# bdaiinstitute/vlfm

Hardware: AMD Instinct MI355X
Metric: env-steps/s (VLM+value-map update), 640x480 RGB-D (higher is better)
Workload: dtype f16 ViT-g (f32 accumulate) + f32 Q-Former (split-f16, 22-bit); f32 confidence + f64 value maps; 1 GPU; configs[1] step x resident envs: BLIP-2 ITC + ValueMap+ObstacleMap+sort_waypoints; envs_per_gpu=256, global_envs=256, map=1000x1000 @ 20 px/m, parallelism=env-sharded x1, tuned_gemms=True, vit_gemm=hip:fc1, attention=hip

## Files before the change

### include/vlfm_amd.h

```cpp
#ifndef VLFM_AMD_H
#define VLFM_AMD_H

#include <stddef.h>
#include <stdint.h>

#ifdef __cplusplus
extern "C" {
#endif

typedef enum {
    VLFM_OK = 0,
    VLFM_ERR_INVALID = -1,
    VLFM_ERR_OUTSIDE_MAP = -2,
    VLFM_ERR_INDEX = -3,
    VLFM_ERR_HIP = -4,
    VLFM_ERR_CAPACITY = -5
} vlfm_status;

enum { VLFM_FUSE_DEFAULT = 0, VLFM_FUSE_REPLACE = 1, VLFM_FUSE_EQUAL_WEIGHTING = 2 };

const char* vlfm_last_error(void);
int vlfm_abi_version(void);

int vlfm_profile_enable(int on);
// ... 127 lines not shown
                                int out_dtype, int patch_size, void* stream);

int vlfm_itc_head_batched(const float* d_proj, int batch, int n_query, int proj_dim,
                          const float* d_text, float* d_out, void* stream);

#define VLFM_ITC_MAX_PROMPTS 8
int vlfm_itc_head_multi(const float* d_proj, int batch, int n_query, int proj_dim, const float* d_text_table, int n_text,
                        const int32_t* d_text_index, int n_prompts, float* d_out, void* stream);

int vlfm_layernorm_bias_f16(const void* d_x, const float* d_channel_bias, const void* d_gamma, const void* d_beta,
                            void* d_y, int rows, int dim, float eps, void* stream);

int vlfm_vit_attention_f16(const void* d_qkv, void* d_out, int batch, int tokens, int heads, int head_dim, float scale,
                           void* stream);

int vlfm_gemm_f16_nt(const void* d_x, const void* d_w, const void* d_bias, void* d_c, int m, int n, int k, int epilogue,
                     void* stream);

int vlfm_gemm_f16_pair_f32_nt(const void* d_x, const void* d_w_pair, const void* d_bias_f32, void* d_out, int m, int n_out, int k,
                              void* stream);

int vlfm_qformer_cross_attention_f32(const void* d_q, const void* d_kv_blocks, void* d_out, int batch, int tokens, int queries,
                                     int heads, int k_block0, int v_block0, int m_total, float scale, void* stream);

int vlfm_gemm_f16_tile_order(int m, int n, int group_m, int* out, int capacity_pairs);
int vlfm_gemm_f16_work_items(int m, int n, int grid, int* out, int capacity_pairs);

int vlfm_split_f32_to_f16_pair(const float* d_src, void* d_hi, void* d_lo, long long count, int* d_overflow, void* stream);
int vlfm_gemm_f32_nt(const float* d_x, const float* d_w, const float* d_bias, const float* d_residual, float* d_c, int m, int n,
                     int k, int activation, int precision, const void* d_w_hi, const void* d_w_lo, int* d_overflow, void* stream);


int vlfm_layernorm_rows_f32(const float* d_x, const float* d_gamma, const float* d_beta, float* d_out, int batch, int height,
                            int width, int channels, int window, float eps, void* stream);
int vlfm_window_reverse_add_f32(float* d_x, const float* d_windows, int batch, int height, int width, int channels, int window,
                                void* stream);
int vlfm_dwconv3x3_nhwc_f32(const float* d_x, const float* d_w9c, const float* d_bias, float* d_out, int batch, int height, int width,
                            int channels, void* stream);
int vlfm_window_attention_f32(const float* d_qkv, const float* d_bias_t, float* d_out, long long windows, int tokens, int heads,
                              float scale, void* stream);
int vlfm_layernorm_rows_shifted_f32(const float* d_x, const float* d_gamma, const float* d_beta, float* d_out, int batch, int height,
                                    int width, int channels, int window, float eps, int shift, int pad_zero, void* stream);
int vlfm_window_reverse_add_shifted_f32(float* d_x, const float* d_windows, int batch, int height, int width, int channels, int window,
                                        int shift, void* stream);
int vlfm_window_attention_masked_f32(const float* d_qkv, const float* d_bias_t, const float* d_mask_t, int windows_per_image, float* d_out,
                                     long long windows, int tokens, int heads, float scale, void* stream);
// ... 254 lines not shown
```

### vlfm_amd/_lib.py

```python
from __future__ import annotations

import ctypes
import os
import subprocess
from typing import Optional

_HERE = os.path.dirname(os.path.abspath(__file__))
LIB_PATH = os.path.join(_HERE, "libvlfm_amd.so")
SOURCES = ["value_map.hip", "depth_ingest.hip", "depth_holes.hip", "obstacle_map.hip", "vlm_ops.hip", "vit_attention.hip", "qformer_attention.hip", "detect_ops.hip", "object_cloud.hip", "cloud_query.hip", "gemm_f16.hip", "gemm_f32.hip", "conv_nhwc.hip", "sam_ops.hip", "map_render.hip", "jpeg_codec.hip", "jpeg_entropy.hip", "jpeg_decode.hip", "world_render.hip", "depth_sensor.hip", "depth_filter.hip", "geodesic.hip", "map_planner.hip", "lattice_geodesic.hip", "host.cpp"]

VLFM_OK = 0
VLFM_ERR_INVALID = -1
VLFM_ERR_OUTSIDE_MAP = -2
VLFM_ERR_INDEX = -3
VLFM_ERR_HIP = -4
VLFM_ERR_CAPACITY = -5

FUSION_TYPES = {"default": 0, "replace": 1, "equal_weighting": 2}


class VmPose(ctypes.Structure):
    _fields_ = [("inv_affine", ctypes.c_double * 6), ("row0", ctypes.c_int32), ("col0", ctypes.c_int32),
                ("env", ctypes.c_int32), ("reserved", ctypes.c_int32)]


class IngestParams(ctypes.Structure):
    _fields_ = [("tf", ctypes.c_double * 12), ("depth_scale", ctypes.c_float), ("depth_offset", ctypes.c_float),
                ("depth_max", ctypes.c_float), ("reserved0", ctypes.c_float), ("fx", ctypes.c_double),
                ("fy", ctypes.c_double), ("min_height", ctypes.c_double), ("max_height", ctypes.c_double),
                ("env", ctypes.c_int32), ("scatter", ctypes.c_int32)]


# ... 70 lines not shown
    if os.path.exists(LIB_PATH) and all(os.path.getmtime(LIB_PATH) >= os.path.getmtime(o) for o in objs):
        return LIB_PATH
    cmd = ["hipcc", "--offload-arch=gfx950", "-shared", "-fPIC", "-o", LIB_PATH] + objs
    if verbose:
        print(" ".join(cmd), flush=True)
    subprocess.check_call(cmd)
    return LIB_PATH


_lib: Optional[ctypes.CDLL] = None


def lib() -> ctypes.CDLL:
    global _lib
    if _lib is None:
        if not os.path.exists(LIB_PATH):
            raise ImportError(
                f"{LIB_PATH} is missing: build it with `python -c 'import __graft_entry__ as g; g.build()'` "
                "(hipcc --offload-arch=gfx950).  vlfm_amd has no CPU fallback.")
        L = ctypes.CDLL(LIB_PATH)
        vp, ci, cd = ctypes.c_void_p, ctypes.c_int, ctypes.c_double
        L.vlfm_last_error.restype = ctypes.c_char_p
        L.vlfm_abi_version.restype = ci
        L.vlfm_profile_enable.argtypes = [ci]
        L.vlfm_host_wait_mode.argtypes = [ci]
        L.vlfm_profile_read.argtypes = [ctypes.c_char_p, ctypes.POINTER(cd), ctypes.POINTER(ci)]
        L.vlfm_value_map_pose_params.argtypes = [vp, vp, vp, ci, ci, ci, ci, vp, ctypes.POINTER(ci)]
        L.vlfm_cone_template_host.argtypes = [cd, cd, ci, cd, vp, ci, vp, ci, ctypes.POINTER(ci)]
        L.vlfm_tan_table_host.argtypes = [cd, ci, vp]
        L.vlfm_disc_rows_host.argtypes = [ci, vp]
        L.vlfm_cone_template_build.argtypes = [vp, vp, ci, ci, vp, vp, vp]
        L.vlfm_depth_ingest_batched.argtypes = [vp, ci, ci, ci, vp, vp, vp, ci, ci, vp, vp, vp, vp, vp]
        L.vlfm_selftest_div_exact.argtypes = [vp, ci, cd, vp, vp]
        L.vlfm_hole_scratch_bytes.argtypes = [ci, ci, ci, ci, ci]
        L.vlfm_hole_scratch_bytes.restype = ctypes.c_size_t
        L.vlfm_fill_small_holes_batched.argtypes = [vp, vp, ci, ci, ci, cd, vp, ctypes.c_size_t, ci, ci, vp, vp, vp, vp,
                                                    ci, vp, vp]
        L.vlfm_depth_scatter_holes_batched.argtypes = [vp, ci, ci, ci, vp, vp, vp, vp, ci, ci, vp, vp, vp]
        L.vlfm_fill_small_holes_rig_batched.argtypes = [vp, vp, ci, ci, ci, cd, vp, ctypes.c_size_t, ci, ci, vp, vp, vp, vp,
                                                        ci, vp, vp, ci, vp]
        L.vlfm_depth_scatter_holes_rig_batched.argtypes = [vp, ci, ci, ci, vp, vp, vp, vp, ci, ci, vp, vp, vp, vp]
        L.vlfm_layernorm_bias_f16.argtypes = [vp, vp, vp, vp, vp, ci, ci, ctypes.c_float, vp]
        L.vlfm_vit_attention_f16.argtypes = [vp, vp, ci, ci, ci, ci, ctypes.c_float, vp]
        L.vlfm_gemm_f16_nt.argtypes = [vp, vp, vp, vp, ci, ci, ci, ci, vp]
        L.vlfm_gemm_f16_pair_f32_nt.argtypes = [vp, vp, vp, vp, ci, ci, ci, vp]
        L.vlfm_qformer_cross_attention_f32.argtypes = [vp, vp, vp, ci, ci, ci, ci, ci, ci, ci, ctypes.c_float, vp]
        L.vlfm_gemm_f32_nt.argtypes = [vp, vp, vp, vp, vp, ci, ci, ci, ci, ci, vp, vp, vp, vp]
        L.vlfm_split_f32_to_f16_pair.argtypes = [vp, vp, vp, ctypes.c_longlong, vp, vp]
        L.vlfm_layernorm_rows_f32.argtypes = [vp, vp, vp, vp, ci, ci, ci, ci, ci, ctypes.c_float, vp]
        L.vlfm_window_reverse_add_f32.argtypes = [vp, vp, ci, ci, ci, ci, ci, vp]
        L.vlfm_dwconv3x3_nhwc_f32.argtypes = [vp, vp, vp, vp, ci, ci, ci, ci, vp]
        L.vlfm_window_attention_f32.argtypes = [vp, vp, vp, ctypes.c_longlong, ci, ci, ctypes.c_float, vp]
        L.vlfm_layernorm_rows_shifted_f32.argtypes = [vp, vp, vp, vp, ci, ci, ci, ci, ci, ctypes.c_float, ci, ci, vp]
        L.vlfm_window_reverse_add_shifted_f32.argtypes = [vp, vp, ci, ci, ci, ci, ci, ci, vp]
        L.vlfm_window_attention_masked_f32.argtypes = [vp, vp, vp, ci, vp, ctypes.c_longlong, ci, ci, ctypes.c_float, vp]
        L.vlfm_maxpool2x2_nhwc_f16.argtypes = [vp, vp, ci, ci, ci, ci, vp]
        L.vlfm_conv_nhwc_tile.argtypes = [ci, ci, ci, ci, ctypes.POINTER(ci), ctypes.POINTER(ci)]
        L.vlfm_conv_nhwc_f16.argtypes = [vp, vp, vp, vp, vp, ci, ci, ci, ci, ci, ci, ci, ci, ci, ci, vp]
        L.vlfm_value_map_update_fused_batched.argtypes = [vp, ci, vp, vp, vp, ci, vp, vp, ci, vp, vp, ci, ci, ci, cd, cd,
                                                          ci, ci, vp, vp, vp, vp, vp]
        L.vlfm_value_map_update_rig_batched.argtypes = [vp, ci, vp, vp, vp, ci, ci, ci, vp, vp, vp, ci, ci, ci, ci, ci, vp, vp,
                                                        vp, vp]
        L.vlfm_value_map_sort_waypoints_batched.argtypes = [vp, ci, ci, vp, ci, ci, vp, ci, vp, vp]
        L.vlfm_resample_coeffs_host.argtypes = [ci, ci, vp, vp, ci, ctypes.POINTER(ci)]
        L.vlfm_resample_coeffs_filter_host.argtypes = [ci, ci, ci, vp, vp, ci, ctypes.POINTER(ci)]
        L.vlfm_preprocess_sam_batched.argtypes = [vp, ci, ci, ci, ci, ci, vp, vp, ci, vp, vp, ci, vp, vp, ci, vp, vp, vp]
        L.vlfm_preprocess_rgb_batched.argtypes = [vp, ci, ci, ci, ci, vp, vp, ci, vp, vp, ci, vp, vp, vp, vp, ci, ci, vp]
        L.vlfm_itc_head_batched.argtypes = [vp, ci, ci, ci, vp, vp, vp]
        L.vlfm_itc_head_multi.argtypes = [vp, ci, ci, ci, vp, ci, vp, ci, vp, vp]
# ... 127 lines not shown
```

### vlfm_amd/csrc/host.cpp

```cpp
#include <cmath>
#include <cstdint>
#include <cstring>
#include <mutex>
#include <string>

#include "../../include/vlfm_amd.h"
#include "status.h"

namespace vlfm {
static thread_local std::string g_last_error;
void set_last_error(const char* msg) { g_last_error = msg ? msg : ""; }
}

extern "C" const char* vlfm_last_error(void) { return vlfm::g_last_error.c_str(); }
extern "C" int vlfm_abi_version(void) { return 28; }

namespace {

const double kPi = 3.141592653589793238462643383279502884;

inline long round_half_even(double v) { return std::lrint(v); }

float sin_deg_table(int deg) {
    static float tab[451];
    static std::once_flag once;
    std::call_once(once, [] {
        for (int i = 0; i <= 450; i++) tab[i] = (float)(std::round(std::sin(i * kPi / 180.0) * 1e7) / 1e7);
    });
    return tab[deg];
}

}

extern "C" int vlfm_value_map_pose_params(const double* h_tf, const double* h_yaw, const int32_t* h_env, int n,
                                          int map_size, int pixels_per_meter, int template_size,
                                          vlfm_vm_pose* h_out, int* bad_index) {
    if (!h_tf || !h_out || n < 0 || map_size <= 0 || template_size <= 0)
        return vlfm::fail(VLFM_ERR_INVALID, "value_map_pose_params: bad argument");
// ... 255 lines not shown
```

### vlfm_amd/csrc/qformer_attention.hip

```cpp
#include <hip/hip_runtime.h>
#include <stdint.h>

#include "../../include/vlfm_amd.h"
#include "mfma.h"
#include "profile.h"
#include "status.h"

namespace vlfm {

constexpr int QA_ROWB = 256;
constexpr int QA_MERGE_REGS = 34;
constexpr int QA_MERGE = 3 * QA_MERGE_REGS * 64 * 4;
constexpr int QA_MAX_T = 257, QA_MAX_Q = 32;

struct QaArgs {
    const float* q;
    const float* kv;
    float* out;
    int B, T, Q, heads, k_block0, v_block0, M_total;
    int rows_pad;
    float scale_log2e;
};

struct QaKernel {
    const QaArgs& a;
    unsigned char* smem;
    lds_ptr lds;
    int lane, wave, col, g, voff;

    __device__ QaKernel(const QaArgs& a_, unsigned char* smem_) : a(a_), smem(smem_), lds((lds_ptr)smem_) {
        lane = threadIdx.x & 63;
        wave = __builtin_amdgcn_readfirstlane(threadIdx.x >> 6);
        col = lane & 31;
        g = lane >> 5;
        voff = a.rows_pad * QA_ROWB;
    }
    __device__ inline const unsigned char* block(int block0, int b, int h) const {
        return reinterpret_cast<const unsigned char*>(a.kv + ((size_t)(block0 + h) * (size_t)a.M_total + (size_t)b * (size_t)a.T) * 64);
    }
    __device__ inline void issue_k(const unsigned char* kg, int row0, int n_ins) const {
        const int r4 = lane >> 4, p = lane & 15;
        for (int ins = 0; ins < n_ins; ins++) {
            const int row = row0 + 4 * ins + r4, src_row = min(row, a.T - 1);
            const int dst = __builtin_amdgcn_readfirstlane((row0 + 4 * ins) * QA_ROWB);
            __builtin_amdgcn_global_load_lds((gbl_ptr)(kg + (size_t)src_row * QA_ROWB + ((p ^ (row & 15)) << 4)), lds + dst, 16, 0, 0);
        }
    }
    __device__ inline void issue_v(const unsigned char* vg, int row0, int n_ins) const {
        const int r4 = lane >> 4, p = lane & 15;
        for (int ins = 0; ins < n_ins; ins++) {
            const int row = row0 + 4 * ins + r4, src_row = min(row, a.T - 1);
            const int dst = __builtin_amdgcn_readfirstlane(voff + (row0 + 4 * ins) * QA_ROWB);
            __builtin_amdgcn_global_load_lds((gbl_ptr)(vg + (size_t)src_row * QA_ROWB + ((p ^ (((row >> 2) & 1) << 3)) << 4)),
                                             lds + dst, 16, 0, 0);
        }
    }
    __device__ inline void issue_rows(const unsigned char* kg, const unsigned char* vg, int row0, int n_ins) const {
        issue_k(kg, row0, n_ins);
        issue_v(vg, row0, n_ins);
    }
    __device__ inline void load_q(int b, int h, float (&qn)[32]) const {
        const float* src = a.q + ((size_t)b * a.Q + min(col, a.Q - 1)) * ((size_t)a.heads * 64) + (size_t)h * 64 + 32 * g;
#pragma unroll
        for (int c = 0; c < 8; c++) {
            const floatx4 v = *reinterpret_cast<const floatx4*>(src + 4 * c);
            qn[4 * c] = v[0]; qn[4 * c + 1] = v[1]; qn[4 * c + 2] = v[2]; qn[4 * c + 3] = v[3];
        }
    }
};

__device__ __forceinline__ void qa_item(int w, int heads, int& b, int& h) {
    const int xcd = w & 7, idx = w >> 3;
    b = (idx / heads) * 8 + xcd;
    h = idx % heads;
}

__global__ __launch_bounds__(256) void qformer_cross_attention_kernel(QaArgs a) {
    extern __shared__ __attribute__((aligned(16))) unsigned char smem[];
    QaKernel k(a, smem);
    const int lane = k.lane, wave = k.wave, col = k.col, g = k.g;
    const int n_full = a.T >> 5, n_left = a.T & 31, left_wave = n_full & 3, left_ins = (n_left + 3) >> 2;
    const int stride = gridDim.x;
    const int moff = 2 * k.voff;
    int w = blockIdx.x, b, h;
    qa_item(w, a.heads, b, h);
// ... 132 lines not shown
                }
            }
            if (col < a.Q) {
                const float inv = 1.0f / l;
                float* orow = a.out + ((size_t)b * a.Q + col) * ((size_t)a.heads * 64) + (size_t)h * 64 + 4 * g;
#pragma unroll
                for (int q4 = 0; q4 < 4; q4++) {
                    const floatx4 s0 = {o0[4 * q4] * inv, o0[4 * q4 + 1] * inv, o0[4 * q4 + 2] * inv, o0[4 * q4 + 3] * inv};
                    const floatx4 s1 = {o1[4 * q4] * inv, o1[4 * q4 + 1] * inv, o1[4 * q4 + 2] * inv, o1[4 * q4 + 3] * inv};
                    *reinterpret_cast<floatx4*>(orow + 8 * q4) = s0;
                    *reinterpret_cast<floatx4*>(orow + 32 + 8 * q4) = s1;
                }
            }
            wait_lgkmcnt0();
        }
        asm volatile("" ::: "memory");
        __builtin_amdgcn_s_barrier();
        asm volatile("" ::: "memory");
        if (!more) break;
        w = nw; b = nb; h = nh;
    }
}

}

using namespace vlfm;

extern "C" int vlfm_qformer_cross_attention_f32(const void* d_q, const void* d_kv_blocks, void* d_out, int batch, int tokens,
                                                int queries, int heads, int k_block0, int v_block0, int m_total, float scale,
                                                void* stream) {
    if (batch == 0) return VLFM_OK;
    if (!d_q || !d_kv_blocks || !d_out || batch < 0 || tokens < 1 || tokens > QA_MAX_T || queries < 1 || queries > QA_MAX_Q || heads < 1 ||
        k_block0 < 0 || v_block0 < 0 || (long long)batch * tokens > (long long)m_total)
        return fail(VLFM_ERR_INVALID, "qformer_cross_attention_f32: head width 64, 1-32 queries, 1-257 tokens, batch * tokens <= m_total");
    if ((((uintptr_t)d_q | (uintptr_t)d_kv_blocks | (uintptr_t)d_out) & 15) != 0)
        return fail(VLFM_ERR_INVALID, "qformer_cross_attention_f32: pointers must be 16-byte aligned");
    QaArgs a;
    a.q = (const float*)d_q; a.kv = (const float*)d_kv_blocks; a.out = (float*)d_out;
    a.B = batch; a.T = tokens; a.Q = queries; a.heads = heads; a.k_block0 = k_block0; a.v_block0 = v_block0; a.M_total = m_total;
    a.rows_pad = (tokens + 3) & ~3;
    a.scale_log2e = scale * 1.4426950408889634f;
    const size_t lds = 2 * (size_t)a.rows_pad * QA_ROWB + QA_MERGE;
    const void* fn = reinterpret_cast<const void*>(qformer_cross_attention_kernel);
    static LdsOptIn opt;
    if (!opt.ensure(fn, lds)) return fail(VLFM_ERR_HIP, "qformer_cross_attention_f32: cannot opt in to the LDS size");
    const long long items = (long long)((batch + 7) / 8) * 8 * heads;
    const int n_cu = device_cu_count() & ~7;
    const dim3 grid((unsigned)(items < n_cu ? items : n_cu)), block(256);
    VLFM_TIMED("qformer_cross_attention_kernel", stream);
    VLFM_KLAUNCH(qformer_cross_attention_kernel, grid, block, lds, stream, a);
    return check_launch("qformer_cross_attention_kernel");
}
```

### vlfm_amd/vlm/blip2itm.py

```python
from __future__ import annotations

import hashlib
import math
import os
import re
from dataclasses import dataclass
from typing import Dict, List, Optional, Sequence, Tuple

import numpy as np
import torch
import torch.nn as nn
import torch.nn.functional as F


@dataclass
class Blip2ITCConfig:
    image_size: int = 224
    patch_size: int = 14
    v_hidden: int = 1408
    v_layers: int = 39
    v_heads: int = 16
    v_mlp: int = 6144
    v_ln_eps: float = 1e-6
    q_hidden: int = 768
# ... 162 lines not shown
def _qlinear(x: torch.Tensor, lin_w: torch.Tensor, lin_b, act=None, residual=None) -> torch.Tensor:
    from . import ops

    if (x.is_cuda and x.dtype == torch.float32 and lin_w.dtype == torch.float32 and not torch.is_grad_enabled()
            and x.numel() // x.shape[-1] >= QFORMER_SPLIT_MIN_ROWS and ops.linear_f32_supported(x, lin_w)):
        return ops.linear_f32(x, lin_w, lin_b, act=act, residual=residual, precision="split", owner="blip2")
    y = F.linear(x, lin_w, lin_b)
    if act == "gelu":
        y = F.gelu(y)
    return y if residual is None else y + residual


class _BertAttention(nn.Module):
    def __init__(self, hidden: int, kv_hidden: int, heads: int, eps: float):
        super().__init__()
        self.heads = heads
        self.query = nn.Linear(hidden, hidden)
        self.key = nn.Linear(kv_hidden, hidden)
        self.value = nn.Linear(kv_hidden, hidden)
        self.dense = nn.Linear(hidden, hidden)
        self.LayerNorm = nn.LayerNorm(hidden, eps=eps)
        self._kv_split = None
        self._qkv_fused = None

    def _project_kv_f16(self, kv16: torch.Tensor) -> Tuple[torch.Tensor, torch.Tensor]:
        if self._kv_split is None or self._kv_split[0].device != kv16.device:
            w1, w2, w3 = _exact_split3(torch.cat([self.key.weight, self.value.weight]))
            bias = torch.cat([self.key.bias, self.value.bias]).detach().float()
            self._kv_split = (w1.t(), w2.t(), w3.t(), bias)
        o = _split_gemm(kv16.reshape(-1, kv16.shape[-1]), self._kv_split[:3], self._kv_split[3])
        o = o.view(*kv16.shape[:-1], -1)
        hid = self.key.out_features
        return o[..., :hid], o[..., hid:]

    def forward(self, x: torch.Tensor, kv: Optional[torch.Tensor] = None, mask: Optional[torch.Tensor] = None,
                kv_proj: Optional[Tuple[torch.Tensor, torch.Tensor]] = None, kv_blocks=None) -> torch.Tensor:
        b, n, d = x.shape
        h = self.heads
        if kv_blocks is not None:
            from . import ops

            blocks, tokens, k_block0, v_block0 = kv_blocks
            q = _qlinear(x, self.query.weight, self.query.bias).contiguous()
            a = ops.qformer_cross_attention(q, blocks, tokens, h, k_block0, v_block0, (d // h) ** -0.5)
            return self.LayerNorm(_qlinear(a, self.dense.weight, self.dense.bias, residual=x))
        if kv_proj is not None:
            q = _qlinear(x, self.query.weight, self.query.bias).view(b, n, h, d // h).transpose(1, 2)
            k = kv_proj[0].reshape(b, -1, h, d // h).transpose(1, 2)
            v = kv_proj[1].reshape(b, -1, h, d // h).transpose(1, 2)
        elif kv is None and x.is_cuda and not self.training:
            if self._qkv_fused is None or self._qkv_fused[0].device != x.device or self._qkv_fused[0].dtype != x.dtype:
                self._qkv_fused = (torch.cat([self.query.weight, self.key.weight, self.value.weight]).detach(),
                                   torch.cat([self.query.bias, self.key.bias, self.value.bias]).detach())
            qkv = _qlinear(x, *self._qkv_fused).view(b, n, 3, h, d // h).permute(2, 0, 3, 1, 4)
            q, k, v = qkv[0], qkv[1], qkv[2]
        else:
            q = self.query(x).view(b, n, h, d // h).transpose(1, 2)
            if kv is not None and kv.dtype == torch.float16 and kv.is_cuda and self.key.weight.dtype == torch.float32:
                k, v = self._project_kv_f16(kv)
                src_len = kv.shape[1]
            else:
                src = x if kv is None else kv.to(x.dtype)
                k, v, src_len = self.key(src), self.value(src), src.shape[1]
            k = k.reshape(b, src_len, h, d // h).transpose(1, 2)
            v = v.reshape(b, src_len, h, d // h).transpose(1, 2)
        a = F.scaled_dot_product_attention(q, k, v, attn_mask=mask)
        return self.LayerNorm(_qlinear(a.transpose(1, 2).reshape(b, n, d), self.dense.weight, self.dense.bias,
                                       residual=x))


class _BertFFN(nn.Module):
    def __init__(self, hidden: int, inter: int, eps: float):
        super().__init__()
        self.up = nn.Linear(hidden, inter)
        self.down = nn.Linear(inter, hidden)
        self.LayerNorm = nn.LayerNorm(hidden, eps=eps)

    def forward(self, x: torch.Tensor) -> torch.Tensor:
        hid = _qlinear(x, self.up.weight, self.up.bias, act="gelu")
        return self.LayerNorm(_qlinear(hid, self.down.weight, self.down.bias, residual=x))
# ... 14 lines not shown
    def __init__(self, cfg: Blip2ITCConfig):
        super().__init__()
        c = self.cfg = cfg
        n_patches = (c.image_size // c.patch_size) ** 2
        self.class_embedding = nn.Parameter(torch.zeros(1, 1, c.v_hidden))
        self.position_embedding = nn.Parameter(torch.zeros(1, n_patches + 1, c.v_hidden))
        self.patch_embedding = nn.Conv2d(3, c.v_hidden, c.patch_size, c.patch_size)
        self.blocks = nn.ModuleList([_VitBlock(c) for _ in range(c.v_layers)])
        self.post_layernorm = nn.LayerNorm(c.v_hidden, eps=c.v_ln_eps)
        self.query_tokens = nn.Parameter(torch.zeros(1, c.num_query_tokens, c.q_hidden))
        self.word_embeddings = nn.Embedding(c.vocab_size, c.q_hidden)
        self.position_embeddings = nn.Embedding(c.max_position_embeddings, c.q_hidden)
        self.q_layernorm = nn.LayerNorm(c.q_hidden, eps=c.q_ln_eps)
        self.q_layers = nn.ModuleList([_QFormerLayer(c, i) for i in range(c.q_layers)])
        self.vision_projection = nn.Linear(c.q_hidden, c.proj_dim)
        self.text_projection = nn.Linear(c.q_hidden, c.proj_dim)
        self.deferred_bias = True
        self._deferred_c: Optional[torch.Tensor] = None
        self.split_kv = True
        self.split_kv_min_rows = 32 * 257
        self._kv_all = None
        self.fused_cross_kv = True
        self._kv_pair = None

    def init_random(self, seed: int = 0) -> "Blip2ITCModel":
        dev = self.query_tokens.device
        g = torch.Generator(device=dev).manual_seed(seed)
        with torch.no_grad():
            for p in self.parameters():
                if p.dim() > 1:
                    p.copy_(torch.randn(p.shape, generator=g, device=dev) * 0.02)
                else:
                    p.zero_()
            for m in self.modules():
                if isinstance(m, nn.LayerNorm):
                    m.weight.fill_(1.0)
        self.weights_changed()
        return self

    def weights_changed(self) -> None:
        self._deferred_c = None
        self._kv_all = None
        self._kv_pair = None
        for layer in self.q_layers:
            layer.attention._qkv_fused = None
            if layer.crossattention is not None:
                layer.crossattention._kv_split = None

    def vision_dtype(self) -> torch.dtype:
        return self.patch_embedding.weight.dtype

    def set_precision(self, vision_dtype: torch.dtype = torch.float16) -> "Blip2ITCModel":
        for m in (self.patch_embedding, self.blocks, self.post_layernorm):
            m.to(vision_dtype)
        self.class_embedding.data = self.class_embedding.data.to(vision_dtype)
        self.position_embedding.data = self.position_embedding.data.to(vision_dtype)
        self.weights_changed()
        return self

    def load_hf_state_dict(self, sd: Dict[str, torch.Tensor]) -> None:
        own = dict(self.named_parameters())

        def put(name: str, src: str) -> None:
            with torch.no_grad():
                own[name].copy_(sd[src].to(own[name].dtype).reshape(own[name].shape))

# ... 15 lines not shown
        put("position_embeddings.weight", "embeddings.position_embeddings.weight")
        put("q_layernorm.weight", "qformer.layernorm.weight")
        put("q_layernorm.bias", "qformer.layernorm.bias")
        for i, layer in enumerate(self.q_layers):
            s, d = f"qformer.encoder.layer.{i}.", f"q_layers.{i}."
            atts = [("attention", "attention")] + ([("crossattention", "crossattention")]
                                                   if layer.crossattention is not None else [])
            for a, b in atts:
                for hf, mine in [("attention.query", "query"), ("attention.key", "key"), ("attention.value", "value"),
                                 ("output.dense", "dense"), ("output.LayerNorm", "LayerNorm")]:
                    put(f"{d}{b}.{mine}.weight", f"{s}{a}.{hf}.weight")
                    put(f"{d}{b}.{mine}.bias", f"{s}{a}.{hf}.bias")
            for hf_i, hf_o, mine in [("intermediate", "output", "ffn_text"),
                                     ("intermediate_query", "output_query", "ffn_query")]:
                put(f"{d}{mine}.up.weight", f"{s}{hf_i}.dense.weight")
                put(f"{d}{mine}.up.bias", f"{s}{hf_i}.dense.bias")
                put(f"{d}{mine}.down.weight", f"{s}{hf_o}.dense.weight")
                put(f"{d}{mine}.down.bias", f"{s}{hf_o}.dense.bias")
                put(f"{d}{mine}.LayerNorm.weight", f"{s}{hf_o}.LayerNorm.weight")
                put(f"{d}{mine}.LayerNorm.bias", f"{s}{hf_o}.LayerNorm.bias")
        for n in ("vision_projection", "text_projection"):
            put(n + ".weight", n + ".weight")
            put(n + ".bias", n + ".bias")

    def load_lavis_state_dict(self, sd: Dict[str, torch.Tensor], vit_sd: Optional[Dict[str, torch.Tensor]] = None) -> None:
        c = self.cfg
        sd = {(k[len("module."):] if k.startswith("module.") else k): v for k, v in sd.items()}
        vit = {("visual_encoder." + k): v for k, v in (vit_sd or {}).items()}
        overlap = set(vit) & set(sd)
        if overlap:
            raise KeyError(f"the vision tower is given twice (e.g. {sorted(overlap)[:2]})")
        src = {**sd, **vit}
        own = dict(self.named_parameters())
        used, fed = set(), set()

        def take(key: str) -> torch.Tensor:
            if key not in src:
                raise KeyError(f"LAVIS state dict lacks {key}" + ("" if vit_sd is not None or not key.startswith("visual_encoder.")
                                                                 else " (blip2_pretrained.pth does not carry the frozen ViT: "
                                                                      "pass eva_vit_g.pth as the vision checkpoint)"))
            used.add(key)
            return src[key]

        def put(name: str, value: torch.Tensor) -> None:
            if tuple(value.shape) != tuple(own[name].shape) and value.numel() != own[name].numel():
                raise ValueError(f"{name}: {tuple(own[name].shape)} in the graph, {tuple(value.shape)} in the file")
# ... 71 lines not shown
                x = blk.forward_deferred(x, c[2 * i], c[2 * i + 1])
            return ops.layernorm_bias(x, c[2 * len(self.blocks)], self.post_layernorm.weight, self.post_layernorm.bias,
                                      self.post_layernorm.eps)
        for blk in self.blocks:
            x = blk(x)
        return self.post_layernorm(x)

    def _deferred_constants(self) -> torch.Tensor:
        if self._deferred_c is None or self._deferred_c.device != self.post_layernorm.weight.device:
            rows, run = [], torch.zeros(self.cfg.v_hidden, dtype=torch.float32, device=self.post_layernorm.weight.device)
            for blk in self.blocks:
                rows.append(run.clone())
                run = run + blk.projection.bias.detach().float()
                rows.append(run.clone())
                run = run + blk.fc2.bias.detach().float()
            rows.append(run.clone())
            self._deferred_c = torch.stack(rows).contiguous()
        return self._deferred_c

    def query_features(self, image_tokens: torch.Tensor) -> torch.Tensor:
        split_ok = (self.split_kv and image_tokens.dtype == torch.float16 and image_tokens.is_cuda
                    and image_tokens.shape[0] * image_tokens.shape[1] >= self.split_kv_min_rows)
        enc = image_tokens if split_ok else image_tokens.to(self.q_layernorm.weight.dtype)
        h = self.q_layernorm(self.query_tokens).expand(enc.shape[0], -1, -1)
        fused = split_ok and self._fused_cross_ok(enc)
        blocks = self._project_all_kv_blocks(enc) if fused else None
        proj = self._project_all_kv(enc) if split_ok and not fused else None
        hid, at = self.cfg.q_hidden, 0
        for layer in self.q_layers:
            h = layer.attention(h)
            if layer.crossattention is not None:
                if blocks is not None:
                    h = layer.crossattention(h, kv_blocks=(blocks, enc.shape[1], at // 64, (at + hid) // 64))
                    at += 2 * hid
                elif proj is not None:
                    h = layer.crossattention(h, kv_proj=(proj[..., at:at + hid], proj[..., at + hid:at + 2 * hid]))
                    at += 2 * hid
                else:
                    h = layer.crossattention(h, kv=enc)
            h = layer.ffn_query(h)
        return h

    def _fused_cross_ok(self, tokens16: torch.Tensor) -> bool:
        from . import ops

        c = self.cfg
        return (self.fused_cross_kv and KV_SPLIT_PIECES == 2 and not torch.is_grad_enabled()
                and self.q_layernorm.weight.dtype == torch.float32
                and c.q_hidden % c.q_heads == 0 and c.q_hidden // c.q_heads == ops.QFORMER_ATTENTION_HEAD
                and c.num_query_tokens <= ops.QFORMER_ATTENTION_MAX_QUERIES
                and 1 <= tokens16.shape[1] <= ops.QFORMER_ATTENTION_MAX_TOKENS and c.v_hidden % 64 == 0
                and tokens16.shape[0] * tokens16.shape[1] * c.v_hidden * 2 < (1 << 32))

    def _kv_all_pieces(self, device):
        if self._kv_all is None or self._kv_all[0].device != device:
            cross = [l.crossattention for l in self.q_layers if l.crossattention is not None]
            w = torch.cat([torch.cat([c.key.weight, c.value.weight]) for c in cross])
            bias = torch.cat([torch.cat([c.key.bias, c.value.bias]) for c in cross]).detach().float()
            w1, w2, w3 = _exact_split3(w)
            self._kv_all = (w1.t(), w2.t(), w3.t(), bias)
            self._kv_pair = None
        return self._kv_all

    def _project_all_kv_blocks(self, tokens16: torch.Tensor) -> torch.Tensor:
# ... 314 lines not shown
```

### vlfm_amd/vlm/ops.py

```python
from __future__ import annotations

import ctypes
from typing import Dict, Optional, Tuple

import numpy as np
import torch

from .. import _lib

CLIP_MEAN = (0.48145466, 0.4578275, 0.40821073)
CLIP_STD = (0.26862954, 0.26130258, 0.27577711)
_DTYPE_CODE = {torch.float32: 0, torch.float16: 1, torch.bfloat16: 2}
_coeff_cache: Dict[Tuple[str, int, int], Tuple[torch.Tensor, torch.Tensor, int]] = {}


def _stream() -> int:
    return torch._C._cuda_getCurrentRawStream(torch._C._cuda_getDevice())


def resample_coeffs(in_size: int, out_size: int, bilinear: bool = False) -> Tuple[np.ndarray, np.ndarray, int]:
    bounds = np.zeros((out_size, 2), np.int32)
    cap = out_size * (2 * int(np.ceil(2.0 * max(1.0, in_size / out_size))) + 1)
    kk = np.zeros(cap, np.int32)
    ks = ctypes.c_int(0)
# ... 260 lines not shown


def linear_pair_f32(x: torch.Tensor, w_pair: torch.Tensor, bias: Optional[torch.Tensor] = None,
                    out: Optional[torch.Tensor] = None) -> torch.Tensor:
    assert x.is_cuda and x.dtype == torch.float16 and x.is_contiguous() and x.dim() == 2
    assert w_pair.dtype == torch.float16 and w_pair.is_contiguous() and w_pair.shape[1] == x.shape[1] and w_pair.shape[0] % 128 == 0
    M, K = x.shape
    N = w_pair.shape[0] // 2
    assert bias is None or (bias.dtype == torch.float32 and bias.is_contiguous() and bias.numel() == N)
    assert all(t is None or t.data_ptr() % 16 == 0 for t in (x, w_pair, bias, out)), "linear_pair_f32: 16-byte aligned tensors only"
    if out is None:
        out = torch.empty((N // 64, M, 64), dtype=torch.float32, device=x.device)
    else:
        assert out.dtype == torch.float32 and out.is_contiguous() and out.shape == (N // 64, M, 64) and out.device == x.device
    _lib.check(_lib.lib().vlfm_gemm_f16_pair_f32_nt(x.data_ptr(), w_pair.data_ptr(), bias.data_ptr() if bias is not None else None,
                                                    out.data_ptr(), M, N, K, _stream()), "gemm_f16_pair_f32_nt")
    return out


QFORMER_ATTENTION_MAX_TOKENS, QFORMER_ATTENTION_MAX_QUERIES, QFORMER_ATTENTION_HEAD = 257, 32, 64


def qformer_cross_attention(q: torch.Tensor, kv_blocks: torch.Tensor, tokens: int, heads: int, k_block0: int, v_block0: int,
                            scale: float, out: Optional[torch.Tensor] = None) -> torch.Tensor:
    assert q.is_cuda and q.dtype == torch.float32 and q.is_contiguous() and q.dim() == 3 and q.shape[2] == heads * 64
    assert kv_blocks.dtype == torch.float32 and kv_blocks.is_contiguous() and kv_blocks.dim() == 3 and kv_blocks.shape[2] == 64
    assert kv_blocks.device == q.device and max(k_block0, v_block0) + heads <= kv_blocks.shape[0] and min(k_block0, v_block0) >= 0
    B, Q, _ = q.shape
    if out is None:
        out = torch.empty_like(q)
    else:
        assert out.dtype == torch.float32 and out.is_contiguous() and out.shape[1:] == q.shape[1:] and out.shape[0] >= B
    _lib.check(_lib.lib().vlfm_qformer_cross_attention_f32(q.data_ptr(), kv_blocks.data_ptr(), out.data_ptr(), B, tokens, Q, heads,
                                                           k_block0, v_block0, kv_blocks.shape[1], float(scale), _stream()),
               "qformer_cross_attention_f32")
    return out


VIT_ATTENTION_TOKENS, VIT_ATTENTION_HEADS = 257, (88,)


def vit_attention(qkv: torch.Tensor, batch: int, tokens: int, heads: int, head_dim: int, scale: float) -> torch.Tensor:
    assert qkv.is_cuda and qkv.dtype == torch.float16 and qkv.is_contiguous()
    assert qkv.numel() == batch * tokens * 3 * heads * head_dim
    out = torch.empty((batch * tokens, heads * head_dim), dtype=torch.float16, device=qkv.device)
    _lib.check(_lib.lib().vlfm_vit_attention_f16(qkv.data_ptr(), out.data_ptr(), batch, tokens, heads, head_dim,
                                                 float(scale), _stream()), "vit_attention_f16")
    return out


_ACT32 = {None: 0, "none": 0, "relu": 1, "gelu": 2}
GEMM_F32_PRECISION = {"exact": 0, "split": 1}
_overflow_flags: Dict[tuple, torch.Tensor] = {}
_split_cache: Dict[int, tuple] = {}


def gemm_f32_overflow_flag(device, owner: str = "") -> torch.Tensor:
    d = torch.device(device)
# ... 114 lines not shown
```

Measured before the change: 1758 env-steps/s.

## Hoist input-independent Q-Former layer-0 prefix and add native self-attention kernel

After: 1759 env-steps/s, median of 3. No clear change (+0.0%).

```diff
diff --git a/include/vlfm_amd.h b/include/vlfm_amd.h
--- a/include/vlfm_amd.h
+++ b/include/vlfm_amd.h
@@ -173,6 +173,11 @@
 
 int vlfm_qformer_cross_attention_f32(const void* d_q, const void* d_kv_blocks, void* d_out, int batch, int tokens, int queries,
                                      int heads, int k_block0, int v_block0, int m_total, float scale, void* stream);
+int vlfm_qformer_cross_attention_strided_f32(const void* d_q, long long q_image_stride, const void* d_kv_blocks, void* d_out, int batch,
+                                             int tokens, int queries, int heads, int k_block0, int v_block0, int m_total, float scale,
+                                             void* stream);
+
+int vlfm_qformer_self_attention_f32(const void* d_qkv, void* d_out, int batch, int queries, int heads, float scale, void* stream);
 
 int vlfm_gemm_f16_tile_order(int m, int n, int group_m, int* out, int capacity_pairs);
 int vlfm_gemm_f16_work_items(int m, int n, int grid, int* out, int capacity_pairs);
diff --git a/vlfm_amd/_lib.py b/vlfm_amd/_lib.py
--- a/vlfm_amd/_lib.py
+++ b/vlfm_amd/_lib.py
@@ -8,6 +8,8 @@
 _HERE = os.path.dirname(os.path.abspath(__file__))
 LIB_PATH = os.path.join(_HERE, "libvlfm_amd.so")
 SOURCES = ["value_map.hip", "depth_ingest.hip", "depth_holes.hip", "obstacle_map.hip", "vlm_ops.hip", "vit_attention.hip", "qformer_attention.hip", "detect_ops.hip", "object_cloud.hip", "cloud_query.hip", "gemm_f16.hip", "gemm_f32.hip", "conv_nhwc.hip", "sam_ops.hip", "map_render.hip", "jpeg_codec.hip", "jpeg_entropy.hip", "jpeg_decode.hip", "world_render.hip", "depth_sensor.hip", "depth_filter.hip", "geodesic.hip", "map_planner.hip", "lattice_geodesic.hip", "host.cpp"]
+
+EXPECTED_ABI = 29
 
 VLFM_OK = 0
 VLFM_ERR_INVALID = -1
@@ -124,6 +126,9 @@
         vp, ci, cd = ctypes.c_void_p, ctypes.c_int, ctypes.c_double
         L.vlfm_last_error.restype = ctypes.c_char_p
         L.vlfm_abi_version.restype = ci
+        if L.vlfm_abi_version() != EXPECTED_ABI:
+            raise ImportError(f"{LIB_PATH} has ABI {L.vlfm_abi_version()}, this package expects {EXPECTED_ABI}: rebuild it "
+                              "(`python -c 'import __graft_entry__ as g; g.build()'`)")
         L.vlfm_profile_enable.argtypes = [ci]
         L.vlfm_host_wait_mode.argtypes = [ci]
         L.vlfm_profile_read.argtypes = [ctypes.c_char_p, ctypes.POINTER(cd), ctypes.POINTER(ci)]
@@ -147,6 +152,8 @@
         L.vlfm_gemm_f16_nt.argtypes = [vp, vp, vp, vp, ci, ci, ci, ci, vp]
         L.vlfm_gemm_f16_pair_f32_nt.argtypes = [vp, vp, vp, vp, ci, ci, ci, vp]
         L.vlfm_qformer_cross_attention_f32.argtypes = [vp, vp, vp, ci, ci, ci, ci, ci, ci, ci, ctypes.c_float, vp]
+        L.vlfm_qformer_cross_attention_strided_f32.argtypes = [vp, ctypes.c_longlong, vp, vp, ci, ci, ci, ci, ci, ci, ci, ctypes.c_float, vp]
+        L.vlfm_qformer_self_attention_f32.argtypes = [vp, vp, ci, ci, ci, ctypes.c_float, vp]
         L.vlfm_gemm_f32_nt.argtypes = [vp, vp, vp, vp, vp, ci, ci, ci, ci, ci, vp, vp, vp, vp]
         L.vlfm_split_f32_to_f16_pair.argtypes = [vp, vp, vp, ctypes.c_longlong, vp, vp]
         L.vlfm_layernorm_rows_f32.argtypes = [vp, vp, vp, vp, ci, ci, ci, ci, ci, ctypes.c_float, vp]
diff --git a/vlfm_amd/csrc/host.cpp b/vlfm_amd/csrc/host.cpp
--- a/vlfm_amd/csrc/host.cpp
+++ b/vlfm_amd/csrc/host.cpp
@@ -13,7 +13,7 @@
 }
 
 extern "C" const char* vlfm_last_error(void) { return vlfm::g_last_error.c_str(); }
-extern "C" int vlfm_abi_version(void) { return 28; }
+extern "C" int vlfm_abi_version(void) { return 29; }
 
 namespace {
 
diff --git a/vlfm_amd/csrc/qformer_attention.hip b/vlfm_amd/csrc/qformer_attention.hip
--- a/vlfm_amd/csrc/qformer_attention.hip
+++ b/vlfm_amd/csrc/qformer_attention.hip
@@ -20,6 +20,7 @@
     int B, T, Q, heads, k_block0, v_block0, M_total;
     int rows_pad;
     float scale_log2e;
+    long long q_stride;
 };
 
 struct QaKernel {
@@ -60,7 +61,7 @@
         issue_v(vg, row0, n_ins);
     }
     __device__ inline void load_q(int b, int h, float (&qn)[32]) const {
-        const float* src = a.q + ((size_t)b * a.Q + min(col, a.Q - 1)) * ((size_t)a.heads * 64) + (size_t)h * 64 + 32 * g;
+        const float* src = a.q + (size_t)b * (size_t)a.q_stride + (size_t)min(col, a.Q - 1) * ((size_t)a.heads * 64) + (size_t)h * 64 + 32 * g;
 #pragma unroll
         for (int c = 0; c < 8; c++) {
             const floatx4 v = *reinterpret_cast<const floatx4*>(src + 4 * c);
@@ -239,16 +240,130 @@
     }
 }
 
+constexpr int QS_MAX_Q = 32, QS_WAVES = 2, QS_WG_PER_CU = 3;
+constexpr int QS_MAT = 32 * QA_ROWB;
+static_assert(QS_WAVES * 3 * QS_MAT <= 64 * 1024 && QS_WG_PER_CU * QS_WAVES * 3 * QS_MAT <= 160 * 1024, "static LDS, QS_WG_PER_CU resident");
+
+struct QsArgs {
+    const float* qkv;
+    float* out;
+    int B, Q, heads;
+    float scale_log2e;
+};
+
+__device__ __forceinline__ void qs_fetch(const QsArgs& a, int item, int r4, int p, floatx4 (&st)[3][8]) {
+    const int b = item / a.heads, h = item - b * a.heads;
+    const size_t row_f = (size_t)3 * a.heads * 64;
+    const float* src = a.qkv + (size_t)b * a.Q * row_f + (size_t)h * 64 + 4 * p;
+#pragma unroll
+    for (int m = 0; m < 3; m++)
+#pragma unroll
+        for (int i = 0; i < 8; i++)
+            st[m][i] = *reinterpret_cast<const floatx4*>(src + (size_t)min(4 * i + r4, a.Q - 1) * row_f + (size_t)m * a.heads * 64);
+}
+
+__global__ __launch_bounds__(64 * QS_WAVES) void qformer_self_attention_kernel(QsArgs a) {
+    __shared__ __attribute__((aligned(16))) unsigned char smem_all[QS_WAVES * 3 * QS_MAT];
+    const int lane = threadIdx.x & 63, wave = __builtin_amdgcn_readfirstlane(threadIdx.x >> 6);
+    unsigned char* smem = smem_all + wave * 3 * QS_MAT;
+    const int col = lane & 31, g = lane >> 5, r4 = lane >> 4, p = lane & 15;
+    const int items = a.B * a.heads, stride = gridDim.x * QS_WAVES;
+    int w = blockIdx.x * QS_WAVES + wave;
+    if (w >= items) return;
+
+    floatx4 st[3][8];
+    qs_fetch(a, w, r4, p, st);
+    for (;;) {
+#pragma unroll
+        for (int i = 0; i < 8; i++) {
+            const int row = 4 * i + r4;
+            *reinterpret_cast<floatx4*>(smem + row * QA_ROWB + ((p ^ (row & 15)) << 4)) = st[0][i];
+            *reinterpret_cast<floatx4*>(smem + QS_MAT + row * QA_ROWB + ((p ^ (row & 15)) << 4)) = st[1][i];
+            *reinterpret_cast<floatx4*>(smem + 2 * QS_MAT + row * QA_ROWB + ((p ^ (((row >> 2) & 1) << 3)) << 4)) = st[2][i];
+        }
+        asm volatile("" ::: "memory");
+        __builtin_amdgcn_wave_barrier();
+        const int b = w / a.heads, h = w - b * a.heads;
+        const int nw = w + stride;
+        const bool more = nw < items;
+        if (more) qs_fetch(a, nw, r4, p, st);
+
+        float qf[32], kf[32];
+#pragma unroll
+        for (int c = 0; c < 8; c++) {
+            const int off = col * QA_ROWB + (((8 * g + c) ^ (col & 15)) << 4);
+            const floatx4 q4 = *reinterpret_cast<const floatx4*>(smem + off);
+            const floatx4 k4 = *reinterpret_cast<const floatx4*>(smem + QS_MAT + off);
+            qf[4 * c] = q4[0]; qf[4 * c + 1] = q4[1]; qf[4 * c + 2] = q4[2]; qf[4 * c + 3] = q4[3];
+            kf[4 * c] = k4[0]; kf[4 * c + 1] = k4[1]; kf[4 * c + 2] = k4[2]; kf[4 * c + 3] = k4[3];
+        }
+        floatx16 acc;
+#pragma unroll
+        for (int r = 0; r < 16; r++) acc[r] = 0.f;
+#pragma unroll
+        for (int s = 0; s < 32; s++) acc = __builtin_amdgcn_mfma_f32_32x32x2f32(kf[s], qf[s], acc, 0, 0, 0);
+        float tm = -INFINITY;
+#pragma unroll
+        for (int r = 0; r < 16; r++)
+            if ((r & 3) + 8 * (r >> 2) + 4 * g < a.Q) tm = fmaxf(tm, acc[r] * a.scale_log2e);
+        tm = fmaxf(tm, __shfl_xor(tm, 32, 64));
+        float l = 0.f;
+#pragma unroll
+        for (int r = 0; r < 16; r++) {
+            const float pj = ((r & 3) + 8 * (r >> 2) + 4 * g < a.Q) ? __builtin_amdgcn_exp2f(fmaf(acc[r], a.scale_log2e, -tm)) : 0.f;
+            l += pj;
+            acc[r] = pj;
+        }
+        l += __shfl_xor(l, 32, 64);
+
+        floatx16 o0, o1;
+#pragma unroll
+        for (int r = 0; r < 16; r++) { o0[r] = 0.f; o1[r] = 0.f; }
+        const float* vb = reinterpret_cast<const float*>(smem + 2 * QS_MAT + 4 * g * QA_ROWB);
+        const int c0 = (((col >> 2) ^ (8 * g)) << 2) + (col & 3), c1 = (((8 + (col >> 2)) ^ (8 * g)) << 2) + (col & 3);
+#pragma unroll
+        for (int r = 0; r < 16; r++) {
+            const int ro = ((r & 3) + 8 * (r >> 2)) * 64;
+            o0 = __builtin_amdgcn_mfma_f32_32x32x2f32(vb[ro + c0], acc[r], o0, 0, 0, 0);
+            o1 = __builtin_amdgcn_mfma_f32_32x32x2f32(vb[ro + c1], acc[r], o1, 0, 0, 0);
+        }
+
+        asm volatile("" ::: "memory");
+        __builtin_amdgcn_wave_barrier();
+        const float inv = 1.0f / l;
+#pragma unroll
+        for (int q4 = 0; q4 < 4; q4++) {
+            const floatx4 s0 = {o0[4 * q4] * inv, o0[4 * q4 + 1] * inv, o0[4 * q4 + 2] * inv, o0[4 * q4 + 3] * inv};
+            const floatx4 s1 = {o1[4 * q4] * inv, o1[4 * q4 + 1] * inv, o1[4 * q4 + 2] * inv, o1[4 * q4 + 3] * inv};
+            *reinterpret_cast<floatx4*>(smem + col * QA_ROWB + (((2 * q4 + g) ^ (col & 15)) << 4)) = s0;
+            *reinterpret_cast<floatx4*>(smem + col * QA_ROWB + (((8 + 2 * q4 + g) ^ (col & 15)) << 4)) = s1;
+        }
+        asm volatile("" ::: "memory");
+        __builtin_amdgcn_wave_barrier();
+        float* orow = a.out + (size_t)b * a.Q * ((size_t)a.heads * 64) + (size_t)h * 64 + 4 * p;
+#pragma unroll
+        for (int i = 0; i < 8; i++) {
+            const int row = 4 * i + r4;
+            const floatx4 v = *reinterpret_cast<const floatx4*>(smem + row * QA_ROWB + ((p ^ (row & 15)) << 4));
+            if (row < a.Q) *reinterpret_cast<floatx4*>(orow + (size_t)row * ((size_t)a.heads * 64)) = v;
+        }
+        asm volatile("" ::: "memory");
+        __builtin_amdgcn_wave_barrier();
+        if (!more) break;
+        w = nw;
+    }
+}
+
 }
 
 using namespace vlfm;
 
-extern "C" int vlfm_qformer_cross_attention_f32(const void* d_q, const void* d_kv_blocks, void* d_out, int batch, int tokens,
-                                                int queries, int heads, int k_block0, int v_block0, int m_total, float scale,
-                                                void* stream) {
+extern "C" int vlfm_qformer_cross_attention_strided_f32(const void* d_q, long long q_image_stride, const void* d_kv_blocks, void* d_out,
+                                                        int batch, int tokens, int queries, int heads, int k_block0, int v_block0,
+                                                        int m_total, float scale, void* stream) {
     if (batch == 0) return VLFM_OK;
     if (!d_q || !d_kv_blocks || !d_out || batch < 0 || tokens < 1 || tokens > QA_MAX_T || queries < 1 || queries > QA_MAX_Q || heads < 1 ||
-        k_block0 < 0 || v_block0 < 0 || (long long)batch * tokens > (long long)m_total)
+        k_block0 < 0 || v_block0 < 0 || (long long)batch * tokens > (long long)m_total || q_image_stride < 0 || (q_image_stride & 3) != 0)
         return fail(VLFM_ERR_INVALID, "qformer_cross_attention_f32: head width 64, 1-32 queries, 1-257 tokens, batch * tokens <= m_total");
     if ((((uintptr_t)d_q | (uintptr_t)d_kv_blocks | (uintptr_t)d_out) & 15) != 0)
         return fail(VLFM_ERR_INVALID, "qformer_cross_attention_f32: pointers must be 16-byte aligned");
@@ -257,6 +372,7 @@
     a.B = batch; a.T = tokens; a.Q = queries; a.heads = heads; a.k_block0 = k_block0; a.v_block0 = v_block0; a.M_total = m_total;
     a.rows_pad = (tokens + 3) & ~3;
     a.scale_log2e = scale * 1.4426950408889634f;
+    a.q_stride = q_image_stride;
     const size_t lds = 2 * (size_t)a.rows_pad * QA_ROWB + QA_MERGE;
     const void* fn = reinterpret_cast<const void*>(qformer_cross_attention_kernel);
     static LdsOptIn opt;
@@ -268,3 +384,28 @@
     VLFM_KLAUNCH(qformer_cross_attention_kernel, grid, block, lds, stream, a);
     return check_launch("qformer_cross_attention_kernel");
 }
+
+extern "C" int vlfm_qformer_cross_attention_f32(const void* d_q, const void* d_kv_blocks, void* d_out, int batch, int tokens,
+                                                int queries, int heads, int k_block0, int v_block0, int m_total, float scale,
+                                                void* stream) {
+    return vlfm_qformer_cross_attention_strided_f32(d_q, (long long)queries * heads * 64, d_kv_blocks, d_out, batch, tokens, queries, heads,
+                                                    k_block0, v_block0, m_total, scale, stream);
+}
+
+extern "C" int vlfm_qformer_self_attention_f32(const void* d_qkv, void* d_out, int batch, int queries, int heads, float scale,
+                                               void* stream) {
+    if (batch == 0) return VLFM_OK;
+    if (!d_qkv || !d_out || batch < 0 || queries < 1 || queries > QS_MAX_Q || heads < 1 || (long long)batch * heads >= (1LL << 30))
+        return fail(VLFM_ERR_INVALID, "qformer_self_attention_f32: head width 64, 1-32 queries, batch * heads < 2^30");
+    if ((((uintptr_t)d_qkv | (uintptr_t)d_out) & 15) != 0)
+        return fail(VLFM_ERR_INVALID, "qformer_self_attention_f32: pointers must be 16-byte aligned");
+    QsArgs a;
+    a.qkv = (const float*)d_qkv; a.out = (float*)d_out;
+    a.B = batch; a.Q = queries; a.heads = heads;
+    a.scale_log2e = scale * 1.4426950408889634f;
+    const long long wgs = ((long long)batch * heads + QS_WAVES - 1) / QS_WAVES, most = (long long)QS_WG_PER_CU * device_cu_count();
+    const dim3 grid((unsigned)(wgs < most ? wgs : most)), block(64 * QS_WAVES);
+    VLFM_TIMED("qformer_self_attention_kernel", stream);
+    VLFM_KLAUNCH(qformer_self_attention_kernel, grid, block, 0, stream, a);
+    return check_launch("qformer_self_attention_kernel");
+}
diff --git a/vlfm_amd/vlm/blip2itm.py b/vlfm_amd/vlm/blip2itm.py
--- a/vlfm_amd/vlm/blip2itm.py
+++ b/vlfm_amd/vlm/blip2itm.py
@@ -208,6 +208,15 @@
         self.LayerNorm = nn.LayerNorm(hidden, eps=eps)
         self._kv_split = None
         self._qkv_fused = None
+        self.native_self_attention = True
+
+    def _native_self_ok(self, qkv: torch.Tensor, mask) -> bool:
+        from . import ops
+
+        b, n, d3 = qkv.shape
+        return (self.native_self_attention and mask is None and qkv.is_cuda and qkv.dtype == torch.float32
+                and not torch.is_grad_enabled() and d3 == 3 * self.heads * ops.QFORMER_ATTENTION_HEAD
+                and 1 <= n <= ops.QFORMER_ATTENTION_MAX_QUERIES and b * self.heads < (1 << 30))
 
     def _project_kv_f16(self, kv16: torch.Tensor) -> Tuple[torch.Tensor, torch.Tensor]:
         if self._kv_split is None or self._kv_split[0].device != kv16.device:
@@ -220,28 +229,43 @@
         return o[..., :hid], o[..., hid:]
 
     def forward(self, x: torch.Tensor, kv: Optional[torch.Tensor] = None, mask: Optional[torch.Tensor] = None,
-                kv_proj: Optional[Tuple[torch.Tensor, torch.Tensor]] = None, kv_blocks=None) -> torch.Tensor:
+                kv_proj: Optional[Tuple[torch.Tensor, torch.Tensor]] = None, kv_blocks=None,
+                q_shared: Optional[torch.Tensor] = None, native_self: bool = False) -> torch.Tensor:
         b, n, d = x.shape
         h = self.heads
         if kv_blocks is not None:
             from . import ops
 
             blocks, tokens, k_block0, v_block0 = kv_blocks
-            q = _qlinear(x, self.query.weight, self.query.bias).contiguous()
-            a = ops.qformer_cross_attention(q, blocks, tokens, h, k_block0, v_block0, (d // h) ** -0.5)
+            if q_shared is not None:
+                a = ops.qformer_cross_attention(q_shared, blocks, tokens, h, k_block0, v_block0, (d // h) ** -0.5, shared_batch=b)
+            else:
+                q = _qlinear(x, self.query.weight, self.query.bias).contiguous()
+                a = ops.qformer_cross_attention(q, blocks, tokens, h, k_block0, v_block0, (d // h) ** -0.5)
             return self.LayerNorm(_qlinear(a, self.dense.weight, self.dense.bias, residual=x))
+        if q_shared is not None:
+            assert kv_proj is not None or kv is not None
+            q = q_shared.expand(b, -1, -1).view(b, n, h, d // h).transpose(1, 2)
         if kv_proj is not None:
-            q = _qlinear(x, self.query.weight, self.query.bias).view(b, n, h, d // h).transpose(1, 2)
+            if q_shared is None:
+                q = _qlinear(x, self.query.weight, self.query.bias).view(b, n, h, d // h).transpose(1, 2)
             k = kv_proj[0].reshape(b, -1, h, d // h).transpose(1, 2)
             v = kv_proj[1].reshape(b, -1, h, d // h).transpose(1, 2)
         elif kv is None and x.is_cuda and not self.training:
             if self._qkv_fused is None or self._qkv_fused[0].device != x.device or self._qkv_fused[0].dtype != x.dtype:
                 self._qkv_fused = (torch.cat([self.query.weight, self.key.weight, self.value.weight]).detach(),
                                    torch.cat([self.query.bias, self.key.bias, self.value.bias]).detach())
-            qkv = _qlinear(x, *self._qkv_fused).view(b, n, 3, h, d // h).permute(2, 0, 3, 1, 4)
+            qkv = _qlinear(x, *self._qkv_fused)
+            if native_self and self._native_self_ok(qkv, mask):
+                from . import ops
+
+                a = ops.qformer_self_attention(qkv.contiguous(), h, (d // h) ** -0.5)
+                return self.LayerNorm(_qlinear(a, self.dense.weight, self.dense.bias, residual=x))
+            qkv = qkv.view(b, n, 3, h, d // h).permute(2, 0, 3, 1, 4)
             q, k, v = qkv[0], qkv[1], qkv[2]
         else:
-            q = self.query(x).view(b, n, h, d // h).transpose(1, 2)
+            if q_shared is None:
+                q = self.query(x).view(b, n, h, d // h).transpose(1, 2)
             if kv is not None and kv.dtype == torch.float16 and kv.is_cuda and self.key.weight.dtype == torch.float32:
                 k, v = self._project_kv_f16(kv)
                 src_len = kv.shape[1]
@@ -302,6 +326,8 @@
         self._kv_all = None
         self.fused_cross_kv = True
         self._kv_pair = None
+        self.hoist_query_prefix = True
+        self._prefix = None
 
     def init_random(self, seed: int = 0) -> "Blip2ITCModel":
         dev = self.query_tokens.device
@@ -322,6 +348,7 @@
         self._deferred_c = None
         self._kv_all = None
         self._kv_pair = None
+        self._prefix = None
         for layer in self.q_layers:
             layer.attention._qkv_fused = None
             if layer.crossattention is not None:
@@ -383,6 +410,7 @@
         for n in ("vision_projection", "text_projection"):
             put(n + ".weight", n + ".weight")
             put(n + ".bias", n + ".bias")
+        self.weights_changed()
 
     def load_lavis_state_dict(self, sd: Dict[str, torch.Tensor], vit_sd: Optional[Dict[str, torch.Tensor]] = None) -> None:
         c = self.cfg
@@ -500,24 +528,46 @@
         split_ok = (self.split_kv and image_tokens.dtype == torch.float16 and image_tokens.is_cuda
                     and image_tokens.shape[0] * image_tokens.shape[1] >= self.split_kv_min_rows)
         enc = image_tokens if split_ok else image_tokens.to(self.q_layernorm.weight.dtype)
-        h = self.q_layernorm(self.query_tokens).expand(enc.shape[0], -1, -1)
+        prefix = self._query_prefix() if self._hoist_ok() else None
+        h = None if prefix is not None else self.q_layernorm(self.query_tokens).expand(enc.shape[0], -1, -1)
         fused = split_ok and self._fused_cross_ok(enc)
         blocks = self._project_all_kv_blocks(enc) if fused else None
         proj = self._project_all_kv(enc) if split_ok and not fused else None
         hid, at = self.cfg.q_hidden, 0
-        for layer in self.q_layers:
-            h = layer.attention(h)
+        for i, layer in enumerate(self.q_layers):
+            q_shared = None
+            if i == 0 and prefix is not None:
+                h, q_shared = prefix[0].expand(enc.shape[0], -1, -1), prefix[1]
+            else:
+                h = layer.attention(h, native_self=True)
             if layer.crossattention is not None:
                 if blocks is not None:
-                    h = layer.crossattention(h, kv_blocks=(blocks, enc.shape[1], at // 64, (at + hid) // 64))
+                    h = layer.crossattention(h, kv_blocks=(blocks, enc.shape[1], at // 64, (at + hid) // 64), q_shared=q_shared)
                     at += 2 * hid
                 elif proj is not None:
-                    h = layer.crossattention(h, kv_proj=(proj[..., at:at + hid], proj[..., at + hid:at + 2 * hid]))
+                    h = layer.crossattention(h, kv_proj=(proj[..., at:at + hid], proj[..., at + hid:at + 2 * hid]), q_shared=q_shared)
                     at += 2 * hid
                 else:
-                    h = layer.crossattention(h, kv=enc)
+                    h = layer.crossattention(h, kv=enc, q_shared=q_shared)
             h = layer.ffn_query(h)
         return h
+
+    def _hoist_ok(self) -> bool:
+        return (self.hoist_query_prefix and not self.training and not torch.is_grad_enabled() and self.query_tokens.is_cuda
+                and len(self.q_layers) > 0 and self.q_layers[0].crossattention is not None)
+
+    def _query_prefix(self) -> Tuple[torch.Tensor, torch.Tensor]:
+        w = self.q_layernorm.weight
+        key = (w.device, w.dtype)
+        if self._prefix is not None and self._prefix[0] == key:
+            return self._prefix[1], self._prefix[2]
+        l0 = self.q_layers[0]
+        h1 = l0.attention(self.q_layernorm(self.query_tokens), native_self=True).contiguous()
+        q0 = F.linear(h1, l0.crossattention.query.weight, l0.crossattention.query.bias).contiguous()
+        if not torch.cuda.is_current_stream_capturing():
+            torch.cuda.current_stream(w.device).synchronize()
+            self._prefix = (key, h1, q0)
+        return h1, q0
 
     def _fused_cross_ok(self, tokens16: torch.Tensor) -> bool:
         from . import ops
diff --git a/vlfm_amd/vlm/ops.py b/vlfm_amd/vlm/ops.py
--- a/vlfm_amd/vlm/ops.py
+++ b/vlfm_amd/vlm/ops.py
@@ -306,18 +306,35 @@
 
 
 def qformer_cross_attention(q: torch.Tensor, kv_blocks: torch.Tensor, tokens: int, heads: int, k_block0: int, v_block0: int,
-                            scale: float, out: Optional[torch.Tensor] = None) -> torch.Tensor:
+                            scale: float, out: Optional[torch.Tensor] = None, shared_batch: Optional[int] = None) -> torch.Tensor:
     assert q.is_cuda and q.dtype == torch.float32 and q.is_contiguous() and q.dim() == 3 and q.shape[2] == heads * 64
     assert kv_blocks.dtype == torch.float32 and kv_blocks.is_contiguous() and kv_blocks.dim() == 3 and kv_blocks.shape[2] == 64
     assert kv_blocks.device == q.device and max(k_block0, v_block0) + heads <= kv_blocks.shape[0] and min(k_block0, v_block0) >= 0
     B, Q, _ = q.shape
+    q_stride = Q * heads * 64
+    if shared_batch is not None:
+        assert B == 1 and shared_batch >= 0
+        B, q_stride = int(shared_batch), 0
     if out is None:
-        out = torch.empty_like(q)
+        out = torch.empty((B, Q, heads * 64), dtype=torch.float32, device=q.device)
     else:
         assert out.dtype == torch.float32 and out.is_contiguous() and out.shape[1:] == q.shape[1:] and out.shape[0] >= B
-    _lib.check(_lib.lib().vlfm_qformer_cross_attention_f32(q.data_ptr(), kv_blocks.data_ptr(), out.data_ptr(), B, tokens, Q, heads,
-                                                           k_block0, v_block0, kv_blocks.shape[1], float(scale), _stream()),
-               "qformer_cross_attention_f32")
+    _lib.check(_lib.lib().vlfm_qformer_cross_attention_strided_f32(q.data_ptr(), q_stride, kv_blocks.data_ptr(), out.data_ptr(), B, tokens,
+                                                                   Q, heads, k_block0, v_block0, kv_blocks.shape[1], float(scale),
+                                                                   _stream()), "qformer_cross_attention_f32")
+    return out
+
+
+def qformer_self_attention(qkv: torch.Tensor, heads: int, scale: float, out: Optional[torch.Tensor] = None) -> torch.Tensor:
+    assert qkv.is_cuda and qkv.dtype == torch.float32 and qkv.is_contiguous() and qkv.dim() == 3 and qkv.shape[2] == 3 * heads * 64
+    B, Q, _ = qkv.shape
+    assert 1 <= Q <= QFORMER_ATTENTION_MAX_QUERIES
+    if out is None:
+        out = torch.empty((B, Q, heads * 64), dtype=torch.float32, device=qkv.device)
+    else:
+        assert out.dtype == torch.float32 and out.is_contiguous() and out.shape == (B, Q, heads * 64) and out.device == qkv.device
+    _lib.check(_lib.lib().vlfm_qformer_self_attention_f32(qkv.data_ptr(), out.data_ptr(), B, Q, heads, float(scale), _stream()),
+               "qformer_self_attention_f32")
     return out
 
 
```
